# Hello1024/shared-tensor

Hardware: AMD Instinct MI355X
Metric: async-DP tokens/sec GPT-2-small (higher is better)
Workload: dtype bf16; 1 GPU; model=gpt2-small, global_batch=64, seq_len=1024, parallelism=async-dp1, codec=1bit, n_params=124439808, paramsync=n/a at n_gpus=1 (no links)

## Files before the change

build.py:

```python
#!/usr/bin/env python3
import argparse
import hashlib
import os
import subprocess
import sysconfig

ROOT = os.path.dirname(os.path.abspath(__file__))
CSRC = os.path.join(ROOT, "sharedtensor_amd", "csrc")
OUT = os.path.join(ROOT, "sharedtensor_amd", "_core.so")
BUILD = os.path.join(ROOT, "build")

SOURCES = [
    "codec_cpu.cpp",
    "engine.cpp",
    "rccl_transport.cpp",
    "hip_kernels.hip",
    "grad_clip_kernels.hip",
    "optim_group_kernels.hip",
    "ln_kernels.hip",
    "add_ln_kernels.hip",
    "add_rms_kernels.hip",
    "ce_kernels.hip",
    "ce_opts_kernels.hip",
    "gelu_kernels.hip",
    "bias_grad_kernels.hip",
    "swiglu_kernels.hip",
    "rope_kernels.hip",
    "bindings.cpp",
]

HEADERS = ["ce_common.h", "common.h", "codec_cpu.h", "device_util.h", "engine.h", "gelu_math.h", "hip_api.h",
           "optim_step.h", "rccl_transport.h"]


def pybind11_include():
    import pybind11
    return pybind11.get_include()


def build(force=False, debug=False, verbose=True):
    os.makedirs(BUILD, exist_ok=True)
    py_inc = sysconfig.get_paths()["include"]
    rocm = os.environ.get("ROCM_PATH", "/opt/rocm")
    hipcc = os.path.join(rocm, "bin", "hipcc")
    cxxflags = [
        "--offload-arch=gfx950",
        "-std=c++20",
        "-O3" if not debug else "-O0",
        "-g" if debug else "",
        "-fPIC",
        "-DSHAMD_WITH_HIP",
        f"-I{CSRC}",
        f"-I{py_inc}",
        f"-I{pybind11_include()}",
        f"-I{rocm}/include",
        "-Wno-unused-result",
        "-fvisibility=hidden",
        "-DNDEBUG" if not debug else "",
        "-parallel-jobs=4",
    ]
    cxxflags = [f for f in cxxflags if f]

    h = hashlib.sha256()
    for f in SOURCES + HEADERS:
        with open(os.path.join(CSRC, f), "rb") as fh:
            h.update(fh.read())
    h.update(" ".join(cxxflags).encode())
    stamp = os.path.join(BUILD, "core.stamp")
    digest = h.hexdigest()
    if not force and os.path.exists(OUT) and os.path.exists(stamp):
        with open(stamp) as fh:
            if fh.read().strip() == digest:
                if verbose:
                    print(f"[build.py] {OUT} up to date")
                return OUT

    objs = []
    procs = []
    for src in SOURCES:
        obj = os.path.join(BUILD, src.replace("/", "_") + ".o")
        objs.append(obj)
        cmd = [hipcc, "-c", os.path.join(CSRC, src), "-o", obj] + cxxflags
        if verbose:
            print("[build.py]", " ".join(cmd))
        procs.append(subprocess.Popen(cmd))
    rc = 0
    for p in procs:
        rc |= p.wait()
    if rc:
        raise RuntimeError("hipcc compilation failed")

    link = [hipcc, "-shared", "-fPIC", "-o", OUT] + objs + [
        f"-L{rocm}/lib", "-lamdhip64", "-lrccl", "-pthread",
        f"-Wl,-rpath,{rocm}/lib",
    ]
    if verbose:
        print("[build.py]", " ".join(link))
    subprocess.check_call(link)
    nm = subprocess.run(["nm", "-C", "-u", OUT], capture_output=True, text=True)
    bad = [l for l in nm.stdout.splitlines() if "shamd::" in l]
    if bad:
        raise RuntimeError("unresolved engine symbols:\n" + "\n".join(bad))
    with open(stamp, "w") as fh:
        fh.write(digest)
    if verbose:
        print(f"[build.py] built {OUT}")
    return OUT


if __name__ == "__main__":
    ap = argparse.ArgumentParser()
    ap.add_argument("--force", action="store_true")
    ap.add_argument("--debug", action="store_true")
    args = ap.parse_args()
    build(force=args.force, debug=args.debug)
```

sharedtensor_amd/csrc/bindings.cpp:

```cpp
#include <pybind11/pybind11.h>
#include <pybind11/stl.h>

#include <array>

#include "codec_cpu.h"
#include "engine.h"
#include "rccl_transport.h"

namespace py = pybind11;
using namespace shamd;

namespace {

py::tuple py_cpu_encode(int codec, uintptr_t delta, int64_t n, double scale_in,
                        uintptr_t payload_out) {
  Codec c = static_cast<Codec>(codec);
  float* d = reinterpret_cast<float*>(delta);
  float scale = scale_in < 0 ? cpu_compute_scale(c, d, n)
                             : static_cast<float>(scale_in);
  cpu_quantize(c, d, n, scale, reinterpret_cast<uint8_t*>(payload_out));
  return py::make_tuple(scale, payload_bytes(c, n));
}

void py_cpu_apply(int codec, uintptr_t payload, int64_t n, double scale,
// ... 236 lines not shown
      .def_readwrite("reconnect", &Config::reconnect)
      .def_readwrite("preserve_subtree", &Config::preserve_subtree)
      .def_readwrite("keepalive_s", &Config::keepalive_s)
      .def_readwrite("bw_limit", &Config::bw_limit)
      .def_readwrite("min_round_interval_s", &Config::min_round_interval_s)
      .def_readwrite("expected_children", &Config::expected_children)
      .def_readwrite("sizes", &Config::sizes)
      .def_readwrite("explicit_parent", &Config::explicit_parent)
      .def_readwrite("listen_port", &Config::listen_port)
      .def_readwrite("join_timeout_s", &Config::join_timeout_s)
      .def_readwrite("rms_sample_stride", &Config::rms_sample_stride)
      .def_readwrite("lagged_scale", &Config::lagged_scale)
      .def_readwrite("delta_bf16", &Config::delta_bf16)
      .def_readwrite("use_graphs", &Config::use_graphs);

  py::class_<Engine>(m, "Engine")
      .def(py::init<Config>())
      .def("set_values", &Engine::set_values)
      .def("set_link_buffers", &Engine::set_link_buffers)
      .def("start", &Engine::start, py::call_guard<py::gil_scoped_release>())
      .def("add_from", &Engine::add_from,
           py::call_guard<py::gil_scoped_release>())
      .def("copy_to", &Engine::copy_to,
           py::call_guard<py::gil_scoped_release>())
      .def("fused_sgd", &Engine::fused_sgd, py::arg("mom"), py::arg("grad"),
           py::arg("lr"), py::arg("momentum"), py::arg("stream"),
           py::arg("clip_state") = 0, py::arg("groups") = 0,
           py::call_guard<py::gil_scoped_release>())
      .def("fused_sgd_bf16", &Engine::fused_sgd_bf16, py::arg("mom"),
           py::arg("grad"), py::arg("shadow"), py::arg("lr"),
           py::arg("momentum"), py::arg("stream"), py::arg("clip_state") = 0, py::arg("groups") = 0,
           py::call_guard<py::gil_scoped_release>())
      .def("fused_adamw", &Engine::fused_adamw, py::arg("mom"),
           py::arg("vel"), py::arg("grad"), py::arg("grad_bf16"),
           py::arg("shadow"), py::arg("lr"), py::arg("beta1"),
           py::arg("beta2"), py::arg("eps"), py::arg("wd"), py::arg("step"),
           py::arg("stream"), py::arg("clip_state") = 0, py::arg("groups") = 0,
           py::call_guard<py::gil_scoped_release>())
      .def("grad_clip_coef", &Engine::grad_clip_coef, py::arg("grad"),
           py::arg("grad_bf16"), py::arg("n"), py::arg("max_norm"),
           py::arg("scratch"), py::arg("state"), py::arg("stream"),
           py::call_guard<py::gil_scoped_release>())
      .def("notify_dirty", &Engine::notify_dirty)
      .def("close", &Engine::close, py::call_guard<py::gil_scoped_release>())
      .def("is_master", &Engine::is_master)
      .def("listen_port", &Engine::listen_port)
      .def("last_error", &Engine::last_error)
      .def("reconnect_count", &Engine::reconnect_count)
      .def("recent_scales_sent", &Engine::recent_scales_sent)
      .def("recent_scales_recv", &Engine::recent_scales_recv)
      .def("link_stats", [](Engine& e) {
        py::list out;
        for (auto& s : e.link_stats()) {
          py::dict d;
          d["rounds_sent"] = s.rounds_sent;
          d["rounds_recv"] = s.rounds_recv;
          d["bytes_sent"] = s.bytes_sent;
          d["bytes_recv"] = s.bytes_recv;
          d["last_scale_sent"] = s.last_scale_sent;
          d["last_scale_recv"] = s.last_scale_recv;
          d["active"] = s.active;
          d["dead"] = s.dead;
          d["peer"] = s.peer;
          d["rccl"] = s.rccl;
          out.append(d);
        }
        return out;
      });

  py::class_<DevCodec>(m, "DevCodec")
      .def(py::init<int, std::vector<int64_t>, int, bool>(), py::arg("codec"),
           py::arg("sizes"), py::arg("device"), py::arg("delta_bf16") = false)
      .def("reduce_scales", &DevCodec::reduce_scales)
      .def("quantize", &DevCodec::quantize, py::arg("delta"),
           py::arg("scales"), py::arg("payload"), py::arg("stream"),
           py::arg("stats") = 0)
      .def("finalize_scales", &DevCodec::finalize_scales)
      .def("apply", &DevCodec::apply);
  m.def("gpu_add_scatter", &py_gpu_add_scatter, py::arg("src"), py::arg("n"),
        py::arg("alpha"), py::arg("dsts"), py::arg("stream"),
        py::arg("delta_bf16") = false);
  m.def("gpu_fused_sgd", &py_gpu_fused_sgd, py::arg("mom"), py::arg("grad"),
        py::arg("lr"), py::arg("mu"), py::arg("n"), py::arg("dsts"),
        py::arg("stream"), py::arg("delta_bf16") = false,
        py::arg("clip_state") = 0, py::arg("groups") = 0);
  m.def("gpu_fused_sgd_bf16", &py_gpu_fused_sgd_bf16, py::arg("mom"),
        py::arg("grad"), py::arg("shadow"), py::arg("lr"), py::arg("mu"),
        py::arg("n"), py::arg("dsts"), py::arg("stream"),
        py::arg("delta_bf16") = false, py::arg("clip_state") = 0, py::arg("groups") = 0);
  m.def("gpu_fused_adamw", &py_gpu_fused_adamw, py::arg("mom"),
        py::arg("vel"), py::arg("grad"), py::arg("grad_bf16"),
        py::arg("shadow"), py::arg("lr"), py::arg("beta1"), py::arg("beta2"),
        py::arg("eps"), py::arg("wd"), py::arg("inv_bc1"), py::arg("inv_bc2"),
        py::arg("n"), py::arg("dsts"), py::arg("stream"),
        py::arg("delta_bf16") = false, py::arg("clip_state") = 0, py::arg("groups") = 0);
  m.def("gpu_grad_clip_coef", &py_gpu_grad_clip_coef, py::arg("grad"),
        py::arg("grad_bf16"), py::arg("n"), py::arg("max_norm"),
        py::arg("scratch"), py::arg("state"), py::arg("stream"));
  m.attr("GRAD_CLIP_MAX_BLOCKS") = GRAD_CLIP_MAX_BLOCKS;
  m.def("build_group_table", &build_group_table, py::arg("n"),
        py::arg("seg_end"), py::arg("seg_group"), py::arg("lr_scale"),
        py::arg("weight_decay"));
  m.attr("GROUP_MAX_SEGMENTS") = GROUP_MAX_SEGMENTS;
  m.attr("GROUP_TILE") = GROUP_TILE;
  m.attr("GROUP_GRID_BLOCKS") = GROUP_GRID_BLOCKS;
  m.def("gpu_snapshot_capture", &py_gpu_snapshot_capture, py::arg("values"),
        py::arg("delta"), py::arg("out"), py::arg("n"), py::arg("stream"),
        py::arg("delta_bf16") = false);
  m.def("gpu_add_delta_scatter", &py_gpu_add_delta_scatter, py::arg("src"),
        py::arg("n"), py::arg("dsts"), py::arg("stream"),
        py::arg("delta_bf16") = false);
  m.def("rccl_loopback_payload", &rccl_loopback_payload,
        "Self ncclSend/ncclRecv of a real payload on one device (1-rank "
        "comm): executes the non-blocking enqueue ordering + stream polling "
        "the 2-GPU xGMI links use and verifies the moved bytes.");
  m.def("rccl_self_test", &rccl_self_test,
        py::call_guard<py::gil_scoped_release>());

  m.def("gelu_fwd", [](uintptr_t x, uintptr_t y, int64_t n, uintptr_t stream) {
    hip_gelu_fwd(reinterpret_cast<const void*>(x), reinterpret_cast<void*>(y),
                 n, reinterpret_cast<hipStream_t>(stream));
  });
  m.def("gelu_bwd", [](uintptr_t dy, uintptr_t x, uintptr_t dx, int64_t n,
                       uintptr_t stream) {
    hip_gelu_bwd(reinterpret_cast<const void*>(dy),
                 reinterpret_cast<const void*>(x),
                 reinterpret_cast<void*>(dx), n,
                 reinterpret_cast<hipStream_t>(stream));
  });

  m.def("bias_grad_partial_floats", &hip_bias_grad_partial_floats);
  m.def("bias_grad_sweep_rows", &hip_bias_grad_sweep_rows);
  m.def("gelu_bwd_colsum", [](uintptr_t dy, uintptr_t x, uintptr_t dx,
                              uintptr_t db, uintptr_t partial, int64_t R,
                              int64_t C, uintptr_t stream) {
    hip_gelu_bwd_colsum(reinterpret_cast<const void*>(dy),
                        reinterpret_cast<const void*>(x),
                        reinterpret_cast<void*>(dx),
                        reinterpret_cast<void*>(db),
                        reinterpret_cast<float*>(partial), R, C,
                        reinterpret_cast<hipStream_t>(stream));
  });
  m.def("pack3_colsum", [](uintptr_t s0, uintptr_t s1, uintptr_t s2,
                           uintptr_t dst, uintptr_t db, uintptr_t partial,
                           int64_t R, int64_t C, uintptr_t stream) {
    hip_pack3_colsum(reinterpret_cast<const void*>(s0),
                     reinterpret_cast<const void*>(s1),
                     reinterpret_cast<const void*>(s2),
                     reinterpret_cast<void*>(dst),
                     reinterpret_cast<void*>(db),
                     reinterpret_cast<float*>(partial), R, C,
                     reinterpret_cast<hipStream_t>(stream));
  });

  m.def("ce_fwd", [](uintptr_t logits, uintptr_t targets, uintptr_t loss,
                     uintptr_t row_m, uintptr_t row_lse, int64_t R, int64_t V,
                     uintptr_t stream) {
    hip_ce_fwd(reinterpret_cast<const void*>(logits),
               reinterpret_cast<const int32_t*>(targets),
               reinterpret_cast<float*>(loss), reinterpret_cast<float*>(row_m),
               reinterpret_cast<float*>(row_lse), R, V,
               reinterpret_cast<hipStream_t>(stream));
  });
  m.def("ce_bwd", [](uintptr_t logits, uintptr_t targets, uintptr_t row_lse,
                     uintptr_t dlogits, uintptr_t gscale_dev, double inv_r,
                     int64_t R, int64_t V, uintptr_t stream,
                     bool skip_if_unit) {
    hip_ce_bwd(reinterpret_cast<const void*>(logits),
               reinterpret_cast<const int32_t*>(targets),
               reinterpret_cast<const float*>(row_lse),
               reinterpret_cast<void*>(dlogits),
               reinterpret_cast<const float*>(gscale_dev),
               static_cast<float>(inv_r), R, V, skip_if_unit,
               reinterpret_cast<hipStream_t>(stream));
  }, py::arg("logits"), py::arg("targets"), py::arg("row_lse"),
     py::arg("dlogits"), py::arg("gscale_dev"), py::arg("inv_r"),
     py::arg("R"), py::arg("V"), py::arg("stream"),
     py::arg("skip_if_unit") = false);
  m.def("ce_fwd_grad", [](uintptr_t logits, uintptr_t targets, uintptr_t loss,
                          uintptr_t row_lse, uintptr_t dlogits, double inv_r,
                          int64_t R, int64_t V, uintptr_t stream) {
    hip_ce_fwd_grad(reinterpret_cast<const void*>(logits),
                    reinterpret_cast<const int32_t*>(targets),
                    reinterpret_cast<float*>(loss),
                    reinterpret_cast<float*>(row_lse),
                    reinterpret_cast<void*>(dlogits),
                    static_cast<float>(inv_r), R, V,
                    reinterpret_cast<hipStream_t>(stream));
  });
  m.def("ce_fwd_grad_max_v", &hip_ce_fwd_grad_max_v);

  m.attr("CE_OPT_STATE_BYTES") = static_cast<int>(sizeof(CeOptState));
  m.def("ce_opts_scan", [](uintptr_t targets, int64_t R, int64_t V,
                           int32_t ignore_index, bool has_ignore,
                           uintptr_t state, uintptr_t stream) {
    hip_ce_opts_scan(reinterpret_cast<const int32_t*>(targets), R, V,
                     CeOpts{ignore_index, has_ignore, 0.f, 0.f},
                     reinterpret_cast<CeOptState*>(state),
                     reinterpret_cast<hipStream_t>(stream));
  }, py::arg("targets"), py::arg("R"), py::arg("V"), py::arg("ignore_index"),
     py::arg("has_ignore"), py::arg("state"), py::arg("stream"));
  m.def("ce_opts_fwd_grad", [](uintptr_t logits, uintptr_t targets,
                               uintptr_t loss, uintptr_t row_lse,
                               uintptr_t dlogits, uintptr_t state, int64_t R,
                               int64_t V, int32_t ignore_index,
                               bool has_ignore, double label_smoothing,
                               double z_loss, uintptr_t stream) {
    hip_ce_opts_fwd_grad(reinterpret_cast<const void*>(logits),
                         reinterpret_cast<const int32_t*>(targets),
                         reinterpret_cast<float*>(loss),
                         reinterpret_cast<float*>(row_lse),
                         reinterpret_cast<void*>(dlogits),
                         reinterpret_cast<const CeOptState*>(state),
                         CeOpts{ignore_index, has_ignore,
                                static_cast<float>(label_smoothing),
                                static_cast<float>(z_loss)},
                         R, V, reinterpret_cast<hipStream_t>(stream));
  }, py::arg("logits"), py::arg("targets"), py::arg("loss"),
     py::arg("row_lse"), py::arg("dlogits"), py::arg("state"), py::arg("R"),
     py::arg("V"), py::arg("ignore_index"), py::arg("has_ignore"),
     py::arg("label_smoothing"), py::arg("z_loss"), py::arg("stream"));
  m.def("ce_opts_fwd", [](uintptr_t logits, uintptr_t targets, uintptr_t loss,
                          uintptr_t row_lse, int64_t R, int64_t V,
                          int32_t ignore_index, bool has_ignore,
                          double label_smoothing, double z_loss,
                          uintptr_t stream) {
    hip_ce_opts_fwd(reinterpret_cast<const void*>(logits),
                    reinterpret_cast<const int32_t*>(targets),
                    reinterpret_cast<float*>(loss),
                    reinterpret_cast<float*>(row_lse),
                    CeOpts{ignore_index, has_ignore,
                           static_cast<float>(label_smoothing),
                           static_cast<float>(z_loss)},
                    R, V, reinterpret_cast<hipStream_t>(stream));
  }, py::arg("logits"), py::arg("targets"), py::arg("loss"),
     py::arg("row_lse"), py::arg("R"), py::arg("V"), py::arg("ignore_index"),
     py::arg("has_ignore"), py::arg("label_smoothing"), py::arg("z_loss"),
     py::arg("stream"));
  m.def("ce_opts_bwd", [](uintptr_t logits, uintptr_t targets,
                          uintptr_t row_lse, uintptr_t dlogits,
                          uintptr_t gscale_dev, uintptr_t state, int64_t R,
                          int64_t V, int32_t ignore_index, bool has_ignore,
                          double label_smoothing, double z_loss,
                          uintptr_t stream, bool skip_if_unit) {
    hip_ce_opts_bwd(reinterpret_cast<const void*>(logits),
                    reinterpret_cast<const int32_t*>(targets),
                    reinterpret_cast<const float*>(row_lse),
                    reinterpret_cast<void*>(dlogits),
                    reinterpret_cast<const float*>(gscale_dev),
                    reinterpret_cast<const CeOptState*>(state),
                    CeOpts{ignore_index, has_ignore,
                           static_cast<float>(label_smoothing),
                           static_cast<float>(z_loss)},
                    R, V, skip_if_unit, reinterpret_cast<hipStream_t>(stream));
  }, py::arg("logits"), py::arg("targets"), py::arg("row_lse"),
     py::arg("dlogits"), py::arg("gscale_dev"), py::arg("state"), py::arg("R"),
     py::arg("V"), py::arg("ignore_index"), py::arg("has_ignore"),
     py::arg("label_smoothing"), py::arg("z_loss"), py::arg("stream"),
     py::arg("skip_if_unit") = false);

  m.def("ln_fwd", [](uintptr_t x, uintptr_t w, uintptr_t b, uintptr_t y,
                     uintptr_t mean, uintptr_t rstd, int64_t R, int C,
                     double eps, uintptr_t stream) {
    hip_ln_fwd(reinterpret_cast<const void*>(x),
               reinterpret_cast<const void*>(w),
               reinterpret_cast<const void*>(b), reinterpret_cast<void*>(y),
               reinterpret_cast<float*>(mean), reinterpret_cast<float*>(rstd),
               R, C, static_cast<float>(eps),
               reinterpret_cast<hipStream_t>(stream));
  });
  m.def("colsum_bf16", [](uintptr_t x, uintptr_t out, int64_t R, int C,
                          uintptr_t stream) {
    hip_colsum_bf16(reinterpret_cast<const void*>(x),
                    reinterpret_cast<float*>(out), R, C,
                    reinterpret_cast<hipStream_t>(stream));
  });
  m.def("swiglu_fwd", [](uintptr_t x1, uintptr_t x3, uintptr_t y, int64_t n,
                         uintptr_t stream) {
    hip_swiglu_fwd(reinterpret_cast<const void*>(x1),
                   reinterpret_cast<const void*>(x3),
                   reinterpret_cast<void*>(y), n,
                   reinterpret_cast<hipStream_t>(stream));
  });
  m.def("swiglu_bwd", [](uintptr_t dy, uintptr_t x1, uintptr_t x3,
                         uintptr_t dx1, uintptr_t dx3, int64_t n,
                         uintptr_t stream) {
    hip_swiglu_bwd(reinterpret_cast<const void*>(dy),
                   reinterpret_cast<const void*>(x1),
                   reinterpret_cast<const void*>(x3),
                   reinterpret_cast<void*>(dx1),
                   reinterpret_cast<void*>(dx3), n,
                   reinterpret_cast<hipStream_t>(stream));
  });
  m.def("rope_qk", [](uintptr_t q, uintptr_t k, uintptr_t q_out,
                      uintptr_t k_out, uintptr_t cos, uintptr_t sin,
                      int64_t B, int64_t Hq, int64_t Hkv, int64_t T,
                      int64_t D, std::array<int64_t, 3> q_strides,
                      std::array<int64_t, 3> k_strides,
                      std::array<int64_t, 3> q_out_strides,
                      std::array<int64_t, 3> k_out_strides, bool inverse,
                      uintptr_t stream) {
    auto st = [](const std::array<int64_t, 3>& a) {
      return RopeStrides{a[0], a[1], a[2]};
    };
    hip_rope_qk(reinterpret_cast<const void*>(q),
                reinterpret_cast<const void*>(k),
// ... 126 lines not shown
```

sharedtensor_amd/csrc/hip_api.h:

```cpp
#pragma once

#include <hip/hip_runtime.h>

#include "common.h"

namespace shamd {

inline int64_t align8(int64_t x) { return (x + 7) & ~int64_t(7); }

struct DevTable {
  int64_t* offs = nullptr;
  int64_t* poffs = nullptr;
  int T = 0;
  int64_t n = 0;
  int64_t pe = 0;
};


void hip_reduce_scales(Codec c, const void* delta, bool delta_bf16,
                       const DevTable& tb, void* reduce_buf, float* scales_out,
                       int sample_stride, hipStream_t s);

void hip_quantize(Codec c, void* delta, bool delta_bf16, const DevTable& tb,
                  const float* scales_dev, uint8_t* payload, hipStream_t s,
// ... 6 lines not shown
               const float* scales_dev, float* values, void* d1, void* d2,
               bool delta_bf16, hipStream_t s);

void hip_add_scatter(const float* src, int64_t n, float alpha, float* values,
                     void* d1, void* d2, void* d3, bool delta_bf16,
                     hipStream_t s);

void hip_snapshot_capture(const float* values, void* delta, bool delta_bf16,
                          float* out, int64_t n, hipStream_t s);

void hip_add_delta_scatter(const void* src_delta, bool delta_bf16, int64_t n,
                           float* values, void* d1, void* d2, hipStream_t s);

void hip_fused_sgd(float* mom, const float* grad, float lr, float momentum,
                   int64_t n, float* values, void* d1, void* d2, void* d3,
                   bool delta_bf16, hipStream_t s,
                   const ClipState* clip = nullptr);

void hip_fused_sgd_bf16(float* mom, const uint16_t* grad, uint16_t* shadow,
                        float lr, float momentum, int64_t n, float* values,
                        void* d1, void* d2, void* d3, bool delta_bf16,
                        hipStream_t s, const ClipState* clip = nullptr);

void hip_fused_adamw(float* mom, float* vel, const void* grad, bool grad_bf16,
                     uint16_t* shadow, float lr, float beta1, float beta2,
                     float eps, float wd, float inv_bc1, float inv_bc2,
                     int64_t n, float* values, void* d1, void* d2, void* d3,
                     bool delta_bf16, hipStream_t s,
                     const ClipState* clip = nullptr);

void hip_fused_sgd_grouped(float* mom, const float* grad, float lr,
                           float momentum, int64_t n, float* values, void* d1,
                           void* d2, void* d3, bool delta_bf16, hipStream_t s,
                           const ClipState* clip, const void* table);
void hip_fused_sgd_bf16_grouped(float* mom, const uint16_t* grad,
                                uint16_t* shadow, float lr, float momentum,
                                int64_t n, float* values, void* d1, void* d2,
                                void* d3, bool delta_bf16, hipStream_t s,
                                const ClipState* clip, const void* table);
void hip_fused_adamw_grouped(float* mom, float* vel, const void* grad,
                             bool grad_bf16, uint16_t* shadow, float lr,
                             float beta1, float beta2, float eps,
                             float inv_bc1, float inv_bc2, int64_t n,
                             float* values, void* d1, void* d2, void* d3,
                             bool delta_bf16, hipStream_t s,
                             const ClipState* clip, const void* table);

void hip_grad_clip_coef(const void* grad, bool grad_bf16, int64_t n,
                        double max_norm, double* scratch, ClipState* state,
                        hipStream_t s);

void hip_ln_fwd(const void* x, const void* w, const void* b, void* y,
                float* mean, float* rstd, int64_t R, int C, float eps,
                hipStream_t s);
void hip_ln_bwd(const void* dy, const void* x, const void* w,
                const float* mean, const float* rstd, void* dx, float* dgamma,
                float* dbeta, int64_t R, int C, hipStream_t s);

bool hip_add_ln_supported(int C);
int hip_add_ln_max_blocks();
void hip_add_ln_fwd(const void* x, const void* delta, const void* dbias,
                    const void* w, const void* b, void* x_new, void* y,
                    float* mean, float* rstd, int64_t R, int C, float eps,
                    hipStream_t s);
void hip_add_ln_bwd(const void* dy, const void* x_new, const void* w,
                    const float* mean, const float* rstd, const void* d_x_new,
                    void* dx_total, void* dgamma, void* dbeta, void* ddbias,
                    float* partial, int64_t R, int C, hipStream_t s);

void hip_colsum_bf16(const void* x, float* out, int64_t R, int C,
                     hipStream_t s);

void hip_rms_fwd(const void* x, const void* w, void* y, float* rstd,
                 int64_t R, int C, float eps, hipStream_t s);
void hip_rms_bwd(const void* dy, const void* x, const void* w,
                 const float* rstd, void* dx, float* dgamma, int64_t R, int C,
                 hipStream_t s);

bool hip_add_rms_supported(int C);
int hip_add_rms_max_blocks();
void hip_add_rms_fwd(const void* x, const void* delta, const void* w,
                     void* x_new, void* y, float* rstd, int64_t R, int C,
                     float eps, hipStream_t s);
void hip_add_rms_bwd(const void* dy, const void* x_new, const void* w,
                     const float* rstd, const void* d_x_new, void* dx_total,
                     void* dgamma, float* partial, int64_t R, int C,
                     hipStream_t s);

void hip_ce_fwd(const void* logits, const int32_t* targets, float* loss,
                float* row_m, float* row_lse, int64_t R, int64_t V,
                hipStream_t s);
void hip_ce_bwd(const void* logits, const int32_t* targets,
                const float* row_lse, void* dlogits, const float* gscale_dev,
                float inv_r, int64_t R, int64_t V, bool skip_if_unit,
                hipStream_t s);
int64_t hip_ce_fwd_grad_max_v();
void hip_ce_fwd_grad(const void* logits, const int32_t* targets, float* loss,
                     float* row_lse, void* dlogits, float inv_r, int64_t R,
                     int64_t V, hipStream_t s);

struct CeOptState {
  float inv_count;
  uint32_t n_valid;
  uint32_t n_bad;
  uint32_t pad;
};
struct CeOpts {
  int32_t ignore_index;
  bool has_ignore;
  float eps;
  float z;
};
void hip_ce_opts_scan(const int32_t* targets, int64_t R, int64_t V,
                      const CeOpts& o, CeOptState* state, hipStream_t s);
void hip_ce_opts_fwd_grad(const void* logits, const int32_t* targets,
                          float* loss, float* row_lse, void* dlogits,
                          const CeOptState* state, const CeOpts& o, int64_t R,
                          int64_t V, hipStream_t s);
void hip_ce_opts_fwd(const void* logits, const int32_t* targets, float* loss,
                     float* row_lse, const CeOpts& o, int64_t R, int64_t V,
                     hipStream_t s);
void hip_ce_opts_bwd(const void* logits, const int32_t* targets,
                     const float* row_lse, void* dlogits,
                     const float* gscale_dev, const CeOptState* state,
                     const CeOpts& o, int64_t R, int64_t V, bool skip_if_unit,
                     hipStream_t s);

void hip_swiglu_fwd(const void* x1, const void* x3, void* y, int64_t n,
                    hipStream_t s);
void hip_swiglu_bwd(const void* dy, const void* x1, const void* x3, void* dx1,
                    void* dx3, int64_t n, hipStream_t s);

struct RopeStrides {
  int64_t b = 0, h = 0, t = 0;
};
void hip_rope_qk(const void* q, const void* k, void* q_out, void* k_out,
                 const float* cos, const float* sin, int64_t B, int64_t Hq,
                 int64_t Hkv, int64_t T, int64_t D, const RopeStrides& q_in,
                 const RopeStrides& k_in, const RopeStrides& q_os,
                 const RopeStrides& k_os, bool inverse, hipStream_t s);

void hip_gelu_fwd(const void* x, void* y, int64_t n, hipStream_t s);
void hip_gelu_bwd(const void* dy, const void* x, void* dx, int64_t n,
                  hipStream_t s);

int64_t hip_bias_grad_partial_floats(int64_t N);
int64_t hip_bias_grad_sweep_rows(int64_t R, int64_t N, bool pack);
void hip_gelu_bwd_colsum(const void* dy, const void* x, void* dx, void* db,
                         float* partial, int64_t R, int64_t C, hipStream_t s);
void hip_pack3_colsum(const void* s0, const void* s1, const void* s2,
                      void* dst, void* db, float* partial, int64_t R,
                      int64_t C, hipStream_t s);

}
```

sharedtensor_amd/models/gpt2.py:

```python
from __future__ import annotations

import math
import os
from dataclasses import dataclass
from typing import Optional

import torch
import torch.nn as nn
import torch.nn.functional as F


@dataclass
class GPT2Config:
    vocab_size: int = 50257
    n_layer: int = 12
    n_head: int = 12
    n_embd: int = 768
    block_size: int = 1024
    dropout: float = 0.0
    ignore_index: Optional[int] = None
    label_smoothing: float = 0.0
    z_loss: float = 0.0

    @classmethod
    def small(cls):
        return cls()

    @classmethod
    def tiny(cls):
        return cls(vocab_size=256, n_layer=2, n_head=2, n_embd=64,
                   block_size=64)


FUSE_PROJ_BIAS = True

FUSE_QKV_BIAS_GRAD = True
FUSE_FC_BIAS_GRAD = False


def _flag(env: str, default: bool) -> bool:
    v = os.environ.get(env)
    return default if v is None else v == "1"


def _bias_grad_ok(flag: bool, which: str, x, lin: nn.Linear) -> bool:
    if not (flag and x.is_cuda and x.dtype == torch.bfloat16
            and lin.bias is not None and torch.is_grad_enabled()):
        return False
    from ..ops import fused_bias_grad as fb
    check = fb.can_use_gelu if which == "gelu" else fb.can_use_qkv
    return check(x, lin.weight, lin.bias)


class FusedLayerNorm(nn.LayerNorm):

    def forward(self, x):
        if (x.is_cuda and x.dtype == torch.bfloat16
                and self.weight.dtype == torch.bfloat16):
            from ..ops import fused_ln
            if fused_ln.can_use(x, self.weight):
                return fused_ln.fused_layer_norm(x, self.weight, self.bias,
                                                 self.eps)
            with torch.autocast("cuda", enabled=False):
                return F.layer_norm(x, self.normalized_shape, self.weight,
                                    self.bias, self.eps)
        return super().forward(x)


def _fused_ln_ok(ln: nn.LayerNorm, x: torch.Tensor) -> bool:
    if (x.is_cuda and x.dtype == torch.bfloat16
            and ln.weight.dtype == torch.bfloat16):
        from ..ops import fused_ln
        return fused_ln.can_use(x, ln.weight)
    return False


def add_ln(ln: nn.LayerNorm, x, delta, delta_bias=None):
    if delta is None:
        return x, ln(x)
    if _fused_ln_ok(ln, x):
        from ..ops import fused_ln
        return fused_ln.fused_add_layer_norm(x, delta, ln.weight, ln.bias,
                                             ln.eps, delta_bias)
    x = x + delta
    if delta_bias is not None:
        x = x + delta_bias
    return x, ln(x)


class CausalSelfAttention(nn.Module):
    def __init__(self, cfg: GPT2Config):
        super().__init__()
        assert cfg.n_embd % cfg.n_head == 0
        self.qkv = nn.Linear(cfg.n_embd, 3 * cfg.n_embd)
        self.proj = nn.Linear(cfg.n_embd, cfg.n_embd)
        self.n_head = cfg.n_head
        self.head_dim = cfg.n_embd // cfg.n_head

    def forward(self, x, proj_bias=True):
        B, T, C = x.shape
        if _bias_grad_ok(_flag("SHTENS_FUSED_QKV_BGRAD", FUSE_QKV_BIAS_GRAD),
                         "qkv", x, self.qkv):
            from ..ops import fused_bias_grad
            qkv = F.linear(x, self.qkv.weight, self.qkv.bias.detach())
            q, k, v = fused_bias_grad.qkv_split_bgrad(qkv, self.qkv.bias)
        else:
            q, k, v = self.qkv(x).split(C, dim=2)
        q = q.view(B, T, self.n_head, self.head_dim).transpose(1, 2)
        k = k.view(B, T, self.n_head, self.head_dim).transpose(1, 2)
        v = v.view(B, T, self.n_head, self.head_dim).transpose(1, 2)
        if x.is_cuda:
            from torch.nn.attention import SDPBackend, sdpa_kernel
            with sdpa_kernel([SDPBackend.EFFICIENT_ATTENTION,
                              SDPBackend.FLASH_ATTENTION, SDPBackend.MATH],
                             set_priority=True):
                y = F.scaled_dot_product_attention(q, k, v, is_causal=True)
        else:
            y = F.scaled_dot_product_attention(q, k, v, is_causal=True)
        y = y.transpose(1, 2).contiguous().view(B, T, C)
        if not proj_bias:
            return F.linear(y, self.proj.weight)
        return self.proj(y)


class MLP(nn.Module):
    def __init__(self, cfg: GPT2Config):
        super().__init__()
        self.fc = nn.Linear(cfg.n_embd, 4 * cfg.n_embd)
        self.proj = nn.Linear(4 * cfg.n_embd, cfg.n_embd)

    def forward(self, x, proj_bias=True):
        if _bias_grad_ok(_flag("SHTENS_FUSED_GELU_BGRAD", FUSE_FC_BIAS_GRAD),
                         "gelu", x, self.fc):
            from ..ops import fused_bias_grad
            pre = F.linear(x, self.fc.weight, self.fc.bias.detach())
            h = fused_bias_grad.bias_gelu_bgrad(pre, self.fc.bias)
        else:
            h = F.gelu(self.fc(x), approximate="tanh")
        if not proj_bias:
            return F.linear(h, self.proj.weight)
        return self.proj(h)


class Block(nn.Module):
    def __init__(self, cfg: GPT2Config):
        super().__init__()
        self.ln1 = FusedLayerNorm(cfg.n_embd)
        self.attn = CausalSelfAttention(cfg)
        self.ln2 = FusedLayerNorm(cfg.n_embd)
        self.mlp = MLP(cfg)

    def forward(self, x, delta=None, delta_bias=None, fuse_proj_bias=False):
        x, h = add_ln(self.ln1, x, delta, delta_bias)
        fuse = fuse_proj_bias and _fused_ln_ok(self.ln2, x)
        a = self.attn(h, proj_bias=not fuse)
        x, h = add_ln(self.ln2, x, a, self.attn.proj.bias if fuse else None)
        m = self.mlp(h, proj_bias=not fuse)
        return x, m, (self.mlp.proj.bias if fuse else None)


class GPT2(nn.Module):
    def __init__(self, cfg: GPT2Config):
        super().__init__()
        self.cfg = cfg
        self.wte = nn.Embedding(cfg.vocab_size, cfg.n_embd)
        self.wpe = nn.Embedding(cfg.block_size, cfg.n_embd)
        self.blocks = nn.ModuleList(Block(cfg) for _ in range(cfg.n_layer))
        self.ln_f = FusedLayerNorm(cfg.n_embd)
        self.lm_head = nn.Linear(cfg.n_embd, cfg.vocab_size, bias=False)
        self.lm_head.weight = self.wte.weight
        self.apply(self._init)
        for name, p in self.named_parameters():
            if name.endswith("proj.weight"):
                nn.init.normal_(p, std=0.02 / math.sqrt(2 * cfg.n_layer))

    @staticmethod
    def _init(m):
        if isinstance(m, nn.Linear):
            nn.init.normal_(m.weight, std=0.02)
            if m.bias is not None:
                nn.init.zeros_(m.bias)
        elif isinstance(m, nn.Embedding):
            nn.init.normal_(m.weight, std=0.02)

    def forward(self, idx, targets=None):
        B, T = idx.shape
        pos = torch.arange(T, device=idx.device)
        x = self.wte(idx) + self.wpe(pos)
        delta = delta_bias = None
        for blk in self.blocks:
            x, delta, delta_bias = blk(x, delta, delta_bias,
                                       FUSE_PROJ_BIAS)
        _, x = add_ln(self.ln_f, x, delta, delta_bias)
        logits = self.lm_head(x)
        if targets is None:
            return logits, None
        flat = logits.view(-1, logits.size(-1))
        tgt = targets.reshape(-1)
        cfg = self.cfg
        if cfg.ignore_index is not None or cfg.label_smoothing != 0.0 \
                or cfg.z_loss != 0.0:
            from ..ops import fused_ce
            opts = dict(ignore_index=cfg.ignore_index,
                        label_smoothing=cfg.label_smoothing,
                        z_loss=cfg.z_loss)
            if fused_ce.can_use(flat):
                return logits, fused_ce.fused_cross_entropy(flat, tgt, **opts)
            return logits, fused_ce.cross_entropy_reference(flat.float(), tgt,
                                                            **opts)
        if flat.is_cuda and flat.dtype == torch.bfloat16:
            from ..ops import fused_ce
            if fused_ce.can_use(flat):
                return logits, fused_ce.fused_cross_entropy(flat, tgt)
        loss = F.cross_entropy(flat, tgt)
        return logits, loss

    def num_params(self) -> int:
        return sum(p.numel() for p in self.parameters())
```

Baseline: 808,900 tokens/s.

## Add custom MFMA flash-attention causal forward kernel for head_dim 64

Adds a hand-written HIP flash-attention forward kernel for causal attention with head_dim 64. It uses bf16 MFMA 32x32x16, double-buffered LDS K/V tiles with swizzled layouts, transpose LDS reads for V, and XCD-aware block scheduling. It replaces the PyTorch SDPA forward while keeping the aten efficient-attention backward, fed with the saved LSE. This targets the SDPA forward cost. The risk is a mismatch between the kernel's LSE and output layout and what the aten backward expects, plus an extra transpose view.

New measurement: 818,700 tokens/s (median of 6 runs). +1.2%, better.

```diff
diff --git a/build.py b/build.py
--- a/build.py
+++ b/build.py
@@ -26,6 +26,7 @@
     "bias_grad_kernels.hip",
     "swiglu_kernels.hip",
     "rope_kernels.hip",
+    "attn_kernels.hip",
     "bindings.cpp",
 ]
 
diff --git a/sharedtensor_amd/csrc/attn_kernels.hip b/sharedtensor_amd/csrc/attn_kernels.hip
--- /dev/null
+++ b/sharedtensor_amd/csrc/attn_kernels.hip
@@ -0,0 +1,274 @@
+#include <hip/hip_runtime.h>
+
+#include "device_util.h"
+#include "hip_api.h"
+
+namespace shamd {
+namespace {
+
+typedef __bf16 bf16x8 __attribute__((ext_vector_type(8)));
+typedef __bf16 bf16x4 __attribute__((ext_vector_type(4)));
+typedef float f32x16 __attribute__((ext_vector_type(16)));
+typedef short s16x4 __attribute__((ext_vector_type(4)));
+
+constexpr int kD = 64;
+constexpr int kQW = 32;
+constexpr int kWaves = 4;
+constexpr int kQB = kQW * kWaves;
+constexpr int kKV = 64;
+constexpr int kTileBytes = kKV * kD * 2;
+constexpr int kXcd = 8;
+
+struct AttnStrides {
+  int64_t b, t, h;
+};
+
+__device__ __forceinline__ int k_off(int row, int ch) {
+  return row * 128 + ((ch ^ ((row >> 1) & 7)) << 4);
+}
+__device__ __forceinline__ int v_off(int row, int ch) {
+  return row * 128 + ((ch ^ (((row >> 1) & 1) << 2)) << 4);
+}
+
+__device__ __forceinline__ uint4 load16_or_zero(const uint16_t* p, bool ok) {
+  uint4 z = make_uint4(0, 0, 0, 0);
+  return ok ? *reinterpret_cast<const uint4*>(p) : z;
+}
+
+__device__ __forceinline__ float other_half(float x) {
+  return __shfl_xor(x, 32, 64);
+}
+
+__global__ __launch_bounds__(256)
+    __attribute__((amdgpu_waves_per_eu(4, 4))) void k_attn_fwd_causal_hd64(
+    const uint16_t* __restrict__ q, const uint16_t* __restrict__ k,
+    const uint16_t* __restrict__ v, uint16_t* __restrict__ out,
+    float* __restrict__ lse, int nbh, int H, int T, int nqb, AttnStrides sq,
+    AttnStrides sk, AttnStrides sv, int64_t lse_stride, float scale_log2e) {
+  __shared__ __attribute__((aligned(16))) unsigned char lds[4 * kTileBytes];
+  unsigned char* const ldsK = lds;
+  unsigned char* const ldsV = lds + 2 * kTileBytes;
+
+  const int xcd = blockIdx.x % kXcd;
+  const int slot = blockIdx.x / kXcd;
+  const int bh = (slot / nqb) * kXcd + xcd;
+  if (bh >= nbh) return;
+  const int qb = nqb - 1 - slot % nqb;
+  const int b = bh / H, h = bh % H;
+
+  const int tid = threadIdx.x;
+  const int wave = __builtin_amdgcn_readfirstlane(tid >> 6), lane = tid & 63;
+  const int r = lane & 31, hi = lane >> 5;
+
+  const int q0 = qb * kQB;
+  const int qw0 = q0 + wave * kQW;
+  const int qrow = qw0 + r;
+
+  const uint16_t* qp = q + b * sq.b + h * sq.h;
+  const uint16_t* kp = k + b * sk.b + h * sk.h;
+  const uint16_t* vp = v + b * sv.b + h * sv.h;
+
+  bf16x8 qf[4];
+#pragma unroll
+  for (int ks = 0; ks < 4; ++ks) {
+    uint4 t = load16_or_zero(qp + (int64_t)qrow * sq.t + 16 * ks + 8 * hi,
+                             qrow < T);
+    qf[ks] = __builtin_bit_cast(bf16x8, t);
+  }
+
+  const int skey = tid >> 3, sch = tid & 7;
+  uint4 stK[2], stV[2];
+  auto issue = [&](int kv0) {
+#pragma unroll
+    for (int i = 0; i < 2; ++i) {
+      int key = kv0 + skey + 32 * i;
+      bool ok = key < T;
+      stK[i] = load16_or_zero(kp + (int64_t)key * sk.t + 8 * sch, ok);
+      stV[i] = load16_or_zero(vp + (int64_t)key * sv.t + 8 * sch, ok);
+    }
+  };
+  auto commit = [&](int buf) {
+#pragma unroll
+    for (int i = 0; i < 2; ++i) {
+      int row = skey + 32 * i;
+      *reinterpret_cast<uint4*>(ldsK + buf * kTileBytes + k_off(row, sch)) =
+          stK[i];
+      *reinterpret_cast<uint4*>(ldsV + buf * kTileBytes + v_off(row, sch)) =
+          stV[i];
+    }
+  };
+
+  const int kv_end = min(T, q0 + kQB);
+  const int ntiles = (kv_end + kKV - 1) / kKV;
+
+  f32x16 o[2];
+#pragma unroll
+  for (int nb = 0; nb < 2; ++nb)
+#pragma unroll
+    for (int i = 0; i < 16; ++i) o[nb][i] = 0.f;
+  float m = -INFINITY;
+  float l = 0.f;
+
+  const int grp = lane >> 4, gi = lane & 15;
+  const int tr_q = gi >> 2, tr_p = gi & 3;
+
+  issue(0);
+  commit(0);
+  __syncthreads();
+
+  for (int t = 0; t < ntiles; ++t) {
+    const int cur = t & 1;
+    const int kv0 = t * kKV;
+    const bool more = t + 1 < ntiles;
+    if (more) issue(kv0 + kKV);
+
+    if (kv0 <= qw0 + kQW - 1) {
+      const unsigned char* Kt = ldsK + cur * kTileBytes;
+      const unsigned char* Vt = ldsV + cur * kTileBytes;
+
+      f32x16 s[2];
+#pragma unroll
+      for (int kb = 0; kb < 2; ++kb) {
+#pragma unroll
+        for (int i = 0; i < 16; ++i) s[kb][i] = 0.f;
+#pragma unroll
+        for (int ks = 0; ks < 4; ++ks) {
+          uint4 kk = *reinterpret_cast<const uint4*>(
+              Kt + k_off(32 * kb + r, 2 * ks + hi));
+          s[kb] = __builtin_amdgcn_mfma_f32_32x32x16_bf16(
+              __builtin_bit_cast(bf16x8, kk), qf[ks], s[kb], 0, 0, 0);
+        }
+      }
+
+      if (kv0 + kKV - 1 > qw0) {
+#pragma unroll
+        for (int kb = 0; kb < 2; ++kb)
+#pragma unroll
+          for (int i = 0; i < 16; ++i) {
+            int key = kv0 + 32 * kb + (i & 3) + 8 * (i >> 2) + 4 * hi;
+            if (key > qrow) s[kb][i] = -INFINITY;
+          }
+      }
+
+      float mx = s[0][0];
+#pragma unroll
+      for (int kb = 0; kb < 2; ++kb)
+#pragma unroll
+        for (int i = 0; i < 16; ++i) mx = fmaxf(mx, s[kb][i]);
+      mx = fmaxf(mx, other_half(mx));
+      const float mn = fmaxf(m, mx * scale_log2e);
+      const float alpha = __builtin_amdgcn_exp2f(m - mn);
+      m = mn;
+
+      float rs = 0.f;
+      bf16x8 pf[4];
+#pragma unroll
+      for (int kb = 0; kb < 2; ++kb)
+#pragma unroll
+        for (int i = 0; i < 16; ++i) {
+          float p = __builtin_amdgcn_exp2f(
+              __builtin_fmaf(s[kb][i], scale_log2e, -mn));
+          rs += p;
+          pf[2 * kb + (i >> 3)][i & 7] = (__bf16)p;
+        }
+      l = l * alpha + rs;
+#pragma unroll
+      for (int nb = 0; nb < 2; ++nb)
+#pragma unroll
+        for (int i = 0; i < 16; ++i) o[nb][i] *= alpha;
+
+#pragma unroll
+      for (int nb = 0; nb < 2; ++nb) {
+#pragma unroll
+        for (int ss = 0; ss < 4; ++ss) {
+          bf16x8 vf;
+#pragma unroll
+          for (int jj = 0; jj < 2; ++jj) {
+            int row = 16 * ss + 8 * jj + 4 * (grp >> 1) + tr_q;
+            int ch = 4 * nb + 2 * (grp & 1) + (tr_p >> 1);
+            auto* a = reinterpret_cast<
+                __attribute__((address_space(3))) s16x4*>(
+                (uintptr_t)(Vt + v_off(row, ch) + 8 * (tr_p & 1)));
+            s16x4 tr = __builtin_amdgcn_ds_read_tr16_b64_v4i16(a);
+            bf16x4 tb = __builtin_bit_cast(bf16x4, tr);
+#pragma unroll
+            for (int e = 0; e < 4; ++e) vf[4 * jj + e] = tb[e];
+          }
+          o[nb] = __builtin_amdgcn_mfma_f32_32x32x16_bf16(vf, pf[ss], o[nb], 0,
+                                                          0, 0);
+        }
+      }
+    }
+
+    if (more) commit(cur ^ 1);
+    __syncthreads();
+  }
+
+  l += other_half(l);
+  const float inv = 1.f / l;
+  if (hi == 0 && qrow < T)
+    lse[(int64_t)bh * lse_stride + qrow] =
+        (m + __builtin_amdgcn_logf(l)) * 0.6931471805599453f;
+
+  unsigned char* const Ow = lds + wave * (kQW * 128);
+#pragma unroll
+  for (int nb = 0; nb < 2; ++nb)
+#pragma unroll
+    for (int g = 0; g < 4; ++g) {
+      float f[4];
+#pragma unroll
+      for (int e = 0; e < 4; ++e) f[e] = o[nb][4 * g + e] * inv;
+      *reinterpret_cast<uint2*>(Ow + k_off(r, 4 * nb + g) + 8 * hi) = pack4(f);
+    }
+  __syncthreads();
+  uint16_t* op = out + ((int64_t)b * T * H + h) * kD;
+#pragma unroll
+  for (int pass = 0; pass < 4; ++pass) {
+    int row = pass * 8 + (lane >> 3), ch = lane & 7;
+    uint4 val = *reinterpret_cast<const uint4*>(Ow + k_off(row, ch));
+    int qr = qw0 + row;
+    if (qr < T)
+      *reinterpret_cast<uint4*>(op + (int64_t)qr * H * kD + 8 * ch) = val;
+  }
+}
+
+}
+
+void hip_attn_fwd_causal_hd64(const void* q, const void* k, const void* v,
+                              void* out, float* lse, int64_t B, int64_t H,
+                              int64_t T, const int64_t* qs, const int64_t* ks,
+                              const int64_t* vs, int64_t lse_stride,
+                              float scale, hipStream_t s) {
+  const char* op = "attn_fwd_causal_hd64";
+  if (B <= 0 || H <= 0 || T <= 0)
+    throw std::runtime_error(std::string(op) + ": empty problem");
+  if (!(scale > 0.f) || scale > 3.0e38f)
+    throw std::runtime_error(std::string(op) + ": scale must be positive");
+  if (lse_stride < T)
+    throw std::runtime_error(std::string(op) + ": lse row shorter than T");
+  check_align(q, 16, op, "q");
+  check_align(k, 16, op, "k");
+  check_align(v, 16, op, "v");
+  check_align(out, 16, op, "out");
+  check_align(lse, 4, op, "lse");
+  for (const int64_t* st : {qs, ks, vs})
+    for (int i = 0; i < 3; ++i)
+      if (st[i] < 0 || st[i] % 8)
+        throw std::runtime_error(std::string(op) +
+                                 ": strides must be multiples of 8 elements");
+  const int64_t nqb = (T + kQB - 1) / kQB;
+  const int64_t nbh = B * H;
+  const int64_t grid = (nbh + kXcd - 1) / kXcd * kXcd * nqb;
+  if (grid > 0x7fffffff || T > (1 << 30) || nbh > 0x7fffffff)
+    throw std::runtime_error(std::string(op) + ": problem too large");
+  AttnStrides a{qs[0], qs[1], qs[2]}, bb{ks[0], ks[1], ks[2]},
+      c{vs[0], vs[1], vs[2]};
+  k_attn_fwd_causal_hd64<<<dim3((unsigned)grid), dim3(256), 0, s>>>(
+      static_cast<const uint16_t*>(q), static_cast<const uint16_t*>(k),
+      static_cast<const uint16_t*>(v), static_cast<uint16_t*>(out), lse,
+      (int)nbh, (int)H, (int)T, (int)nqb, a, bb, c, lse_stride,
+      scale * 1.4426950408889634f);
+  HIP_CHECK(hipGetLastError());
+}
+
+}
diff --git a/sharedtensor_amd/csrc/bindings.cpp b/sharedtensor_amd/csrc/bindings.cpp
--- a/sharedtensor_amd/csrc/bindings.cpp
+++ b/sharedtensor_amd/csrc/bindings.cpp
@@ -412,6 +412,25 @@
                      reinterpret_cast<float*>(partial), R, C,
                      reinterpret_cast<hipStream_t>(stream));
   });
+
+  m.def("attn_fwd_causal_hd64",
+        [](uintptr_t q, uintptr_t k, uintptr_t v, uintptr_t out, uintptr_t lse,
+           int64_t B, int64_t H, int64_t T, std::array<int64_t, 3> q_strides,
+           std::array<int64_t, 3> k_strides, std::array<int64_t, 3> v_strides,
+           int64_t lse_stride, double scale, uintptr_t stream) {
+          hip_attn_fwd_causal_hd64(
+              reinterpret_cast<const void*>(q),
+              reinterpret_cast<const void*>(k),
+              reinterpret_cast<const void*>(v), reinterpret_cast<void*>(out),
+              reinterpret_cast<float*>(lse), B, H, T, q_strides.data(),
+              k_strides.data(), v_strides.data(), lse_stride,
+              static_cast<float>(scale),
+              reinterpret_cast<hipStream_t>(stream));
+        },
+        py::arg("q"), py::arg("k"), py::arg("v"), py::arg("out"),
+        py::arg("lse"), py::arg("B"), py::arg("H"), py::arg("T"),
+        py::arg("q_strides"), py::arg("k_strides"), py::arg("v_strides"),
+        py::arg("lse_stride"), py::arg("scale"), py::arg("stream"));
 
   m.def("ce_fwd", [](uintptr_t logits, uintptr_t targets, uintptr_t loss,
                      uintptr_t row_m, uintptr_t row_lse, int64_t R, int64_t V,
diff --git a/sharedtensor_amd/csrc/hip_api.h b/sharedtensor_amd/csrc/hip_api.h
--- a/sharedtensor_amd/csrc/hip_api.h
+++ b/sharedtensor_amd/csrc/hip_api.h
@@ -182,4 +182,11 @@
                       void* dst, void* db, float* partial, int64_t R,
                       int64_t C, hipStream_t s);
 
+void hip_attn_fwd_causal_hd64(const void* q, const void* k, const void* v,
+                              void* out, float* lse, int64_t B, int64_t H,
+                              int64_t T, const int64_t* q_strides,
+                              const int64_t* k_strides,
+                              const int64_t* v_strides, int64_t lse_stride,
+                              float scale, hipStream_t s);
+
 }
diff --git a/sharedtensor_amd/models/gpt2.py b/sharedtensor_amd/models/gpt2.py
--- a/sharedtensor_amd/models/gpt2.py
+++ b/sharedtensor_amd/models/gpt2.py
@@ -37,10 +37,19 @@
 FUSE_QKV_BIAS_GRAD = True
 FUSE_FC_BIAS_GRAD = False
 
+FUSE_ATTN_FWD = True
+
 
 def _flag(env: str, default: bool) -> bool:
     v = os.environ.get(env)
     return default if v is None else v == "1"
+
+
+def _attn_ok(q, k, v) -> bool:
+    if not (_flag("SHTENS_FUSED_ATTN", FUSE_ATTN_FWD) and q.is_cuda):
+        return False
+    from ..ops import fused_attn
+    return fused_attn.can_use(q, k, v)
 
 
 def _bias_grad_ok(flag: bool, which: str, x, lin: nn.Linear) -> bool:
@@ -109,7 +118,10 @@
         q = q.view(B, T, self.n_head, self.head_dim).transpose(1, 2)
         k = k.view(B, T, self.n_head, self.head_dim).transpose(1, 2)
         v = v.view(B, T, self.n_head, self.head_dim).transpose(1, 2)
-        if x.is_cuda:
+        if _attn_ok(q, k, v):
+            from ..ops import fused_attn
+            y = fused_attn.fused_causal_attention(q, k, v)
+        elif x.is_cuda:
             from torch.nn.attention import SDPBackend, sdpa_kernel
             with sdpa_kernel([SDPBackend.EFFICIENT_ATTENTION,
                               SDPBackend.FLASH_ATTENTION, SDPBackend.MATH],
diff --git a/sharedtensor_amd/ops/fused_attn.py b/sharedtensor_amd/ops/fused_attn.py
--- /dev/null
+++ b/sharedtensor_amd/ops/fused_attn.py
@@ -0,0 +1,101 @@
+from __future__ import annotations
+
+import math
+
+import torch
+
+from .. import _core
+
+HEAD_DIM = 64
+
+
+def _sdpa_priority():
+    from torch.nn.attention import SDPBackend, sdpa_kernel
+    return sdpa_kernel([SDPBackend.EFFICIENT_ATTENTION,
+                        SDPBackend.FLASH_ATTENTION, SDPBackend.MATH],
+                       set_priority=True)
+
+
+def _strides_ok(t: torch.Tensor) -> bool:
+    sb, sh, st, sd = t.stride()
+    return (sd == 1 and sb % 8 == 0 and sh % 8 == 0 and st % 8 == 0
+            and min(sb, sh, st) >= 0 and t.data_ptr() % 16 == 0)
+
+
+def can_use(q: torch.Tensor, k: torch.Tensor, v: torch.Tensor) -> bool:
+    if not (q.is_cuda and k.is_cuda and v.is_cuda):
+        return False
+    if not (q.dtype == k.dtype == v.dtype == torch.bfloat16):
+        return False
+    if q.dim() != 4 or q.shape != k.shape or q.shape != v.shape:
+        return False
+    if q.shape[-1] != HEAD_DIM or q.numel() == 0:
+        return False
+    return _strides_ok(q) and _strides_ok(k) and _strides_ok(v)
+
+
+def attn_forward(q, k, v, scale=None, out=None, lse=None):
+    if not can_use(q, k, v):
+        raise ValueError("fused_attn: inputs the kernel does not take "
+                         "(see can_use)")
+    B, H, T, D = q.shape
+    if scale is None:
+        scale = 1.0 / math.sqrt(D)
+    if out is None:
+        out = torch.empty((B, T, H, D), dtype=q.dtype, device=q.device)
+    if lse is None:
+        lse = torch.empty((B, H, T), dtype=torch.float32, device=q.device)
+    if (out.shape != (B, T, H, D) or not out.is_contiguous()
+            or out.dtype != torch.bfloat16):
+        raise ValueError("fused_attn: out must be contiguous (B, T, H, 64) bf16")
+    if (lse.shape != (B, H, T) or not lse.is_contiguous()
+            or lse.dtype != torch.float32):
+        raise ValueError("fused_attn: lse must be contiguous (B, H, T) fp32")
+
+    def bth(t):
+        sb, sh, st, _ = t.stride()
+        return [sb, st, sh]
+
+    s = torch.cuda.current_stream(q.device).cuda_stream
+    _core.attn_fwd_causal_hd64(q.data_ptr(), k.data_ptr(), v.data_ptr(),
+                               out.data_ptr(), lse.data_ptr(), B, H, T,
+                               bth(q), bth(k), bth(v), T, float(scale), s)
+    return out, lse
+
+
+_philox = None
+
+
+def _philox_state():
+    global _philox
+    if _philox is None:
+        _philox = (torch.empty((), dtype=torch.int64),
+                   torch.empty((), dtype=torch.int64))
+    return _philox
+
+
+class _FusedCausalAttn(torch.autograd.Function):
+    @staticmethod
+    def forward(ctx, q, k, v, scale):
+        out, lse = attn_forward(q, k, v, scale)
+        out = out.transpose(1, 2)
+        ctx.save_for_backward(q, k, v, out, lse)
+        ctx.scale = scale
+        return out
+
+    @staticmethod
+    def backward(ctx, dout):
+        q, k, v, out, lse = ctx.saved_tensors
+        seed, offset = _philox_state()
+        with _sdpa_priority():
+            dq, dk, dv, _ = \
+                torch.ops.aten._scaled_dot_product_efficient_attention_backward(
+                    dout, q, k, v, None, out, lse, seed, offset, 0.0,
+                    [True, True, True, False], True, scale=ctx.scale)
+        return dq, dk, dv, None
+
+
+def fused_causal_attention(q, k, v, scale=None):
+    if scale is None:
+        scale = 1.0 / math.sqrt(q.shape[-1])
+    return _FusedCausalAttn.apply(q, k, v, float(scale))
```
